# nanograv/PTMCMCSampler

Hardware: AMD Instinct MI355X
Metric: MH updates/sec (whole node) + ESS/sec, 100-d Gaussian, 64 temps x 4096 walkers per GPU (higher is better)
Workload: dtype f64

## Files before the change

### ptmcmcsampler_amd/csrc/ptmi_cov.hip

```cpp
#include <math.h>
#include <stdlib.h>

#include <type_traits>

#include "ptmi_common.h"

constexpr int WT = 7, WTILE = 16 * WT;
template <bool FUSED>
__global__ __launch_bounds__(256) void welford_kernel(const double *AM, double *mu, double *M2, double *cov, int d, int mem,
                                                     long long iter, int cov_stride_per_walker, int am_epl)
{
    constexpr int PF = 8;
    constexpr int RB = 4;
    __shared__ double sh[2][RB][2][WTILE];
    if (FUSED && blockIdx.y > blockIdx.x) return;
    const int w = (int)blockIdx.z;
    const int ti0 = (int)blockIdx.y * WTILE, tj0 = (int)blockIdx.x * WTILE;
    const int tx = (int)(threadIdx.x & 15), ty = (int)(threadIdx.x >> 4);
    const double *am = AM + (size_t)w * mem * d;
    double *muw = mu + (size_t)w * d, *M2w = M2 + (size_t)w * d * d;
    long long it = iter - mem;
    const bool reset = it == 0;

    const int role = (int)threadIdx.x / WTILE, ridx = (int)threadIdx.x % WTILE;
    const int rel = role == 0 ? ti0 + ridx : tj0 + ridx;
    const bool carrier = role < 2 && rel < d;
    double m = carrier && !reset ? muw[rel] : 0.0;

    double acc[WT][WT];
#pragma unroll
    for (int p = 0; p < WT; ++p)
#pragma unroll
        for (int r = 0; r < WT; ++r) {
            const int i = ti0 + ty + 16 * p, j = tj0 + tx + 16 * r;
            acc[p][r] = (!reset && i < d && j < d) ? M2w[(size_t)i * d + j] : 0.0;
        }
    int bsel = 0;
    for (int ii0 = 0; ii0 < mem; ii0 += PF) {
        double vpre[PF];
#pragma unroll
        for (int u = 0; u < PF; ++u) vpre[u] = (carrier && ii0 + u < mem) ? am[(size_t)(ii0 + u) * d + am_pos(rel < d ? rel : 0, am_epl)] : 0.0;
#pragma unroll
        for (int u0 = 0; u0 < PF; u0 += RB) {
            if (ii0 + u0 >= mem) break;
            if (role < 2) {
#pragma unroll
                for (int u = 0; u < RB; ++u) {
                    double df = 0.0, ev = 0.0;
                    if (carrier && ii0 + u0 + u < mem) {
                        const double v = vpre[u0 + u];
                        df = v - m;
                        if (FUSED) m = m + df * (1.0 / (double)(it + 1 + u));
                        else m += df / (double)(it + 1 + u);
                        ev = v - m;
                    }
                    if (role == 0) sh[bsel][u][0][ridx] = df;
                    else sh[bsel][u][1][ridx] = ev;
                }
            }
            __syncthreads();
#pragma unroll
            for (int u = 0; u < RB; ++u) {
                double dv[WT], evv[WT];
#pragma unroll
                for (int p = 0; p < WT; ++p) dv[p] = sh[bsel][u][0][ty + 16 * p];
#pragma unroll
                for (int r = 0; r < WT; ++r) evv[r] = sh[bsel][u][1][tx + 16 * r];
                if (ii0 + u0 + u < mem) {
#pragma unroll
                    for (int p = 0; p < WT; ++p)
#pragma unroll
                        for (int r = 0; r < WT; ++r) {
                            if (FUSED) acc[p][r] = __builtin_fma(dv[p], evv[r], acc[p][r]);
                            else acc[p][r] += dv[p] * evv[r];
                        }
                }
            }
            const int done = mem - (ii0 + u0) < RB ? mem - (ii0 + u0) : RB;
            it += done;
            bsel ^= 1;
        }
    }
    const double den = (double)(it - 1);
    double *covw = cov ? cov + (size_t)w * cov_stride_per_walker : nullptr;
#pragma unroll
    for (int p = 0; p < WT; ++p)
#pragma unroll
        for (int r = 0; r < WT; ++r) {
            const int i = ti0 + ty + 16 * p, j = tj0 + tx + 16 * r;
            if (i < d && j < d) {
                M2w[(size_t)i * d + j] = acc[p][r];
                if (covw) covw[(size_t)i * d + j] = acc[p][r] / den;
            }
        }
    if (gridDim.x == 1 && role == 0 && carrier) muw[rel] = m;
}

__device__ __forceinline__ double div_by_count(double a, double n, double r)
{
    if (__builtin_fabs(a) < 0x1p-900) return a / n;
    double q = a * r;
    double e = __builtin_fma(-n, q, a);
    q = __builtin_fma(e, r, q);
    e = __builtin_fma(-n, q, a);
    return __builtin_fma(e, r, q);
}
template <int TYN, int TXN, int PR, int PC>
__global__ __launch_bounds__(768) void welford_rows_kernel(const double *AM, double *mu, double *M2, double *cov, int d, int mem, long long iter,
                                                           int cov_stride_per_walker, int am_epl, int nwalkers)
{
#ifndef PTMI_WF_RB
#define PTMI_WF_RB 8
#endif
    constexpr int RB = PTMI_WF_RB, LW = TYN * PR > TXN * PC ? TYN * PR : TXN * PC;
    __shared__ __attribute__((aligned(16))) double sh_all[2][2][RB][2][LW];
    const int tb = (int)threadIdx.x;
    const int slot = tb < 512 ? tb >> 8 : (tb - 512) >> 7;
    const int w = 2 * (int)blockIdx.x + slot;
    const bool wact = w < nwalkers;
    double (*sh)[RB][2][LW] = sh_all[slot];
    const double *am = AM + (size_t)(wact ? w : 0) * mem * d;
    double *muw = mu + (size_t)(wact ? w : 0) * d, *M2w = M2 + (size_t)(wact ? w : 0) * d * d;
    const long long it0 = iter - mem;
    const bool reset = it0 == 0;
    const int t = tb < 512 ? (tb & 255) : 256 + ((tb - 512) & 127);
    const int nb = (mem + RB - 1) / RB;
    if (t >= 256) {
        const int rel = t - 256;
        const bool carrier = rel < d && wact;
        const int pos = am_pos(carrier ? rel : 0, am_epl);
        double m = carrier && !reset ? muw[rel] : 0.0;
        double vc[RB], vn[RB];
        auto load = [&](int b, double (&v)[RB]) {
#pragma unroll
            for (int u = 0; u < RB; ++u) {
                const int row = b * RB + u;
                v[u] = (carrier && row < mem) ? am[(size_t)row * d + pos] : 0.0;
            }
        };
        auto produce = [&](int b, const double (&v)[RB]) {
            const double nl = (double)(it0 + (long long)b * RB + 1 + (t & (RB - 1))), rl = 1.0 / nl;
#pragma unroll
            for (int u = 0; u < RB; ++u) {
                const double n = __shfl(nl, u, RB), r = __shfl(rl, u, RB);
                double df = 0.0, ev = 0.0;
#ifdef PTMI_WF_NOCARRY
                df = v[u] + n; ev = v[u] + r;
#else
                if (b * RB + u < mem) {
                    df = v[u] - m;
                    m += div_by_count(df, n, r);
                    ev = v[u] - m;
                }
#endif
                if (rel < LW) { sh[b & 1][u][0][rel] = carrier ? df : 0.0; sh[b & 1][u][1][rel] = carrier ? ev : 0.0; }
            }
        };
        load(0, vc);
        if (nb > 1) load(1, vn);
        produce(0, vc);
        __syncthreads();
        for (int b = 0; b < nb; ++b) {
            if (b + 1 < nb) {
#pragma unroll
                for (int u = 0; u < RB; ++u) vc[u] = vn[u];
                if (b + 2 < nb) load(b + 2, vn);
                produce(b + 1, vc);
            }
            __syncthreads();
        }
        if (carrier && wact) muw[rel] = m;
        return;
    }
    const int ty = t / TXN, tx = t % TXN;
    const bool live = t < TYN * TXN && wact;
    double acc[PR][PC];
#pragma unroll
    for (int p = 0; p < PR; ++p)
#pragma unroll
        for (int r = 0; r < PC; ++r) {
            const int i = ty * PR + p, j = tx * PC + r;
            acc[p][r] = (live && !reset && i < d && j < d) ? M2w[(size_t)i * d + j] : 0.0;
        }
    __syncthreads();
    for (int b = 0; b < nb; ++b) {
        if (live) {
            double dv[2][PR], ev[2][PC];
            auto rd = [&](int u, int k) {
#pragma unroll
                for (int p = 0; p < PR; ++p) dv[k][p] = sh[b & 1][u][0][ty * PR + p];
#pragma unroll
                for (int r = 0; r < PC; ++r) ev[k][r] = sh[b & 1][u][1][tx * PC + r];
            };
            auto row = [&](int k) {
#pragma unroll
                for (int p = 0; p < PR; ++p)
#pragma unroll
                    for (int r = 0; r < PC; ++r) acc[p][r] += dv[k][p] * ev[k][r];
            };
            rd(0, 0);
#pragma unroll
            for (int u = 0; u < RB; ++u) {
                if (u + 1 < RB) {
                    rd(u + 1, (u + 1) & 1);
                    __builtin_amdgcn_sched_barrier(0);
                }
                row(u & 1);
            }
        }
        __syncthreads();
    }
    if (!live) return;
    const double den = (double)(iter - 1);
    double *covw = cov ? cov + (size_t)w * cov_stride_per_walker : nullptr;
#pragma unroll
    for (int p = 0; p < PR; ++p)
#pragma unroll
        for (int r = 0; r < PC; ++r) {
            const int i = ty * PR + p, j = tx * PC + r;
            if (i < d && j < d) M2w[(size_t)i * d + j] = acc[p][r];
        }
    if (covw) {
#pragma unroll 1
        for (int e = 0; e < PR * PC; ++e) {
            const int i = ty * PR + e / PC, j = tx * PC + e % PC;
            if (i < d && j < d) covw[(size_t)i * d + j] = M2w[(size_t)i * d + j] / den;
        }
    }
}

constexpr int PS_W = 112;
constexpr int ps_rc(bool diag) { return diag ? 32 : 16; }
typedef double ps_d4 __attribute__((ext_vector_type(4)));
__host__ __device__ inline int pool_groups(int d) { return (d + 1 + PS_W - 1) / PS_W; }
static inline int pool_slab(int nwalkers, int d) { const int target = d + 1 <= PS_W ? 512 : 32; const int s = (nwalkers + target - 1) / target; return s < 1 ? 1 : s; }
struct PoolEnt { double wgt; int32_t src; int32_t pad; };
struct PoolRle { const PoolEnt *ent; const int32_t *cnt; };
typedef double ps_d2 __attribute__((ext_vector_type(2)));
constexpr int ps_nt(bool diag, int wv) { return diag ? 7 : (wv == 0 ? 13 : 12); }
__host__ __device__ constexpr int ps_t0(int wv) { return wv == 0 ? 0 : 1 + 12 * wv; }
constexpr int ps_ti(bool diag, int wv, int n) { return diag ? (n < 7 - wv ? wv : 7 - wv) : (ps_t0(wv) + n) / 7; }
constexpr int ps_tj(bool diag, int wv, int n) { return diag ? (n < 7 - wv ? wv + n : n) : (ps_t0(wv) + n) % 7; }
template <bool DIAG, int WV>
__device__ __forceinline__ void ps_mma(const double *Ab, const double *Bb, ps_d4 (&acc)[DIAG ? 7 : 13])
{
#pragma unroll
    for (int k0 = 0; k0 < ps_rc(DIAG); k0 += 4)
#pragma unroll
        for (int n = 0; n < ps_nt(DIAG, WV); ++n)
            acc[n] = __builtin_amdgcn_mfma_f64_16x16x4f64(Ab[k0 * PS_W + 16 * ps_ti(DIAG, WV, n)], Bb[k0 * PS_W + 16 * ps_tj(DIAG, WV, n)], acc[n], 0, 0, 0);
}
template <bool DIAG, int WV>
__device__ __forceinline__ void ps_store(const ps_d4 (&acc)[DIAG ? 7 : 13], double *out, int I, int J, int d, int am_epl, int g, int c)
{
#pragma unroll
    for (int n = 0; n < ps_nt(DIAG, WV); ++n) {
        const int ti = ps_ti(DIAG, WV, n), tj = ps_tj(DIAG, WV, n);
#pragma unroll
        for (int r = 0; r < 4; ++r) {
            const int pi = I * PS_W + 16 * ti + g + 4 * r, pj = J * PS_W + 16 * tj + c;
            if (pi < d && pj <= d && (!(DIAG && ti == tj) || pi <= pj)) {
                const int ci = am_inv(pi, am_epl), cj = pj < d ? am_inv(pj, am_epl) : d;
                const int lo = ci < cj ? ci : cj, hi = ci < cj ? cj : ci;
                out[(size_t)lo * (d + 1) + hi] = acc[n][r];
            }
        }
    }
}
template <bool DIAG, bool RLE, bool PAIR>
__global__ __launch_bounds__(256, 2) void pool_syrk_kernel(const double *rows, long long nrows, int d, const double *shift,
                                                                     long long rows_per_slab, double *part, int am_epl,
                                                                     int shift_epl ,
                                                                     PoolRle rl)
{
    constexpr int NTW = DIAG ? 7 : 13, NA = DIAG ? 1 : 2, PS_RC = ps_rc(DIAG), NU = PS_RC / 4;
    __shared__ double Dl[NA][2][PS_RC][PS_W];
    const int lane = (int)(threadIdx.x & 63), wave = __builtin_amdgcn_readfirstlane((int)(threadIdx.x >> 6));
    const int c = lane & 15, g = lane >> 4;
    const int ng = pool_groups(d);
    int I = (int)blockIdx.x, J = (int)blockIdx.x;
    if (!DIAG) {
        int p = (int)blockIdx.x;
        I = 0;
        while (p >= ng - 1 - I) { p -= ng - 1 - I; ++I; }
        J = I + 1 + p;
    }
    const long long beg = (long long)blockIdx.y * rows_per_slab;
    const int nlist = RLE ? rl.cnt[blockIdx.y] : (int)(beg + rows_per_slab < nrows ? rows_per_slab : nrows - beg);
    const char *slab = (const char *)(rows + beg * d);
    const PoolEnt *ent = RLE ? rl.ent + beg : nullptr;
    ps_d4 acc[NTW];
#pragma unroll
    for (int n = 0; n < NTW; ++n) acc[n] = ps_d4{0.0, 0.0, 0.0, 0.0};
    int offa[DIAG ? 1 : NTW], offb[DIAG ? 1 : NTW];
    if constexpr (!DIAG) {
#pragma unroll
        for (int n = 0; n < NTW; ++n) {
            const int t = ps_t0(wave) + n < 49 ? ps_t0(wave) + n : 48;
            offa[n] = __builtin_amdgcn_readfirstlane(16 * (t / 7));
            offb[n] = __builtin_amdgcn_readfirstlane(16 * (t % 7));
        }
    }
    const int q = 16 * wave + c, r4 = g;
    const bool stager = q < PS_W / 2;
    unsigned colb[NA][2];
    double sh[NA][2], one[NA][2];
    bool dat[NA][2];
    bool plain = true;
#pragma unroll
    for (int a2 = 0; a2 < NA; ++a2)
#pragma unroll
        for (int e = 0; e < 2; ++e) {
            const int p = (a2 == 0 ? I : J) * PS_W + 2 * q + e;
            dat[a2][e] = p < d;
            const int pc = PAIR ? (p - e < d ? p : d - 2 + e) : (p < d ? p : d - 1);
            colb[a2][e] = 8u * (unsigned)pc;
            sh[a2][e] = (stager && p < d) ? shift[am_pos(am_inv(p, am_epl), shift_epl)] : 0.0;
            one[a2][e] = p == d ? 1.0 : 0.0;
            plain = plain && (dat[a2][e] || !stager);
        }
    const bool wave_plain = __all(plain);
    const unsigned rstride = 8u * (unsigned)d;
    ps_d2 v[NA][NU];
    double wg[NU];
    int nsrc[RLE ? NU : 1];
    double nwg[RLE ? NU : 1];
    auto list = [&](int j0) {
        if constexpr (RLE) {
#pragma unroll
            for (int u = 0; u < NU; ++u) {
                const int j = j0 + 4 * u + r4, jc = j < nlist ? j : nlist - 1;
                const ps_d2 e2 = *(const ps_d2 *)(ent + jc);
                nwg[u] = e2.x;
                nsrc[u] = (int)(__double_as_longlong(e2.y) & 0xffffffffll);
            }
        }
    };
    auto fetch = [&](int j0) {
#pragma unroll
        for (int u = 0; u < NU; ++u) {
            const int j = j0 + 4 * u + r4, jc = j < nlist ? j : nlist - 1;
            const unsigned rb = (unsigned)(RLE ? nsrc[u] : jc) * rstride;
            wg[u] = j < nlist ? (RLE ? nwg[u] : 1.0) : 0.0;
#pragma unroll
            for (int a2 = 0; a2 < NA; ++a2) {
                if constexpr (PAIR) v[a2][u] = *(const ps_d2 *)(slab + (rb + colb[a2][0]));
                else {
                    v[a2][u].x = *(const double *)(slab + (rb + colb[a2][0]));
                    v[a2][u].y = *(const double *)(slab + (rb + colb[a2][1]));
                }
            }
        }
    };
    auto stage = [&](int buf) {
        if (!stager) return;
        if (wave_plain) {
#pragma unroll
            for (int a2 = 0; a2 < NA; ++a2)
#pragma unroll
                for (int u = 0; u < NU; ++u) {
                    ps_d2 x;
                    x.x = (v[a2][u].x - sh[a2][0]) * wg[u];
                    x.y = (v[a2][u].y - sh[a2][1]) * wg[u];
                    *(ps_d2 *)&Dl[a2][buf][4 * u + r4][2 * q] = x;
                }
        } else {
#pragma unroll
            for (int a2 = 0; a2 < NA; ++a2)
#pragma unroll
                for (int u = 0; u < NU; ++u) {
                    ps_d2 x;
                    x.x = (dat[a2][0] ? v[a2][u].x - sh[a2][0] : one[a2][0]) * wg[u];
                    x.y = (dat[a2][1] ? v[a2][u].y - sh[a2][1] : one[a2][1]) * wg[u];
                    *(ps_d2 *)&Dl[a2][buf][4 * u + r4][2 * q] = x;
                }
        }
    };
    if (nlist > 0) {
        list(0);
        fetch(0);
        list(PS_RC);
        stage(0);
    }
    __syncthreads();
    int buf = 0;
    for (int j0 = 0; j0 < nlist; j0 += PS_RC) {
        const bool more = j0 + PS_RC < nlist;
        if (more) {
            fetch(j0 + PS_RC);
            list(j0 + 2 * PS_RC);
        }
        const double *Ab = &Dl[0][buf][0][0] + g * PS_W + c, *Bb = &Dl[NA - 1][buf][0][0] + g * PS_W + c;
        if constexpr (DIAG) {
            switch (wave) {
            case 0: ps_mma<DIAG, 0>(Ab, Bb, acc); break;
            case 1: ps_mma<DIAG, 1>(Ab, Bb, acc); break;
            case 2: ps_mma<DIAG, 2>(Ab, Bb, acc); break;
            default: ps_mma<DIAG, 3>(Ab, Bb, acc); break;
            }
        } else {
#pragma unroll
            for (int k0 = 0; k0 < PS_RC; k0 += 4)
#pragma unroll
                for (int n = 0; n < NTW; ++n)
                    if (n < 12 || wave == 0) acc[n] = __builtin_amdgcn_mfma_f64_16x16x4f64(Ab[k0 * PS_W + offa[n]], Bb[k0 * PS_W + offb[n]], acc[n], 0, 0, 0);
        }
        if (more) stage(buf ^ 1);
        __syncthreads();
        buf ^= 1;
    }
    double *out = part + (size_t)blockIdx.y * d * (d + 1);
    if constexpr (DIAG) {
        switch (wave) {
        case 0: ps_store<DIAG, 0>(acc, out, I, J, d, am_epl, g, c); break;
        case 1: ps_store<DIAG, 1>(acc, out, I, J, d, am_epl, g, c); break;
        case 2: ps_store<DIAG, 2>(acc, out, I, J, d, am_epl, g, c); break;
        default: ps_store<DIAG, 3>(acc, out, I, J, d, am_epl, g, c); break;
        }
    } else {
#pragma unroll
        for (int n = 0; n < NTW; ++n) {
            if (!(n < 12 || wave == 0)) continue;
#pragma unroll
            for (int r = 0; r < 4; ++r) {
                const int pi = I * PS_W + offa[n] + g + 4 * r, pj = J * PS_W + offb[n] + c;
                if (pi < d && pj <= d) {
                    const int ci = am_inv(pi, am_epl), cj = pj < d ? am_inv(pj, am_epl) : d;
                    const int lo = ci < cj ? ci : cj, hi = ci < cj ? cj : ci;
                    out[(size_t)lo * (d + 1) + hi] = acc[n][r];
                }
            }
        }
    }
}

__global__ __launch_bounds__(256) void pool_rle_kernel(const AmFlag *flag, long long nrows, long long rows_per_slab, PoolEnt *ent, int32_t *cnt)
{
    constexpr int NG = 8;
    __shared__ int wsum[NG][4], base_s;
    const long long beg = (long long)blockIdx.x * rows_per_slab;
    const long long end = beg + rows_per_slab < nrows ? beg + rows_per_slab : nrows;
    const int lane = (int)(threadIdx.x & 63), wave = (int)(threadIdx.x >> 6);
    if (threadIdx.x == 0) base_s = 0;
    __syncthreads();
    for (long long r0 = beg; r0 < end; r0 += 256 * NG) {
        AmFlag f[NG];
#pragma unroll
        for (int u = 0; u < NG; ++u) { const long long r = r0 + 256 * u + threadIdx.x; f[u] = flag[r < end ? r : end - 1]; }
        unsigned long long m[NG];
#pragma unroll
        for (int u = 0; u < NG; ++u) {
            const long long r = r0 + 256 * u + threadIdx.x;
            m[u] = __ballot(r < end && (f[u] & (AMROW_NEW | AMROW_KEY)) != 0);
            if (lane == 0) wsum[u][wave] = (int)__popcll(m[u]);
        }
        __syncthreads();
        int off = base_s;
#pragma unroll
        for (int u = 0; u < NG; ++u) {
            const long long r = r0 + 256 * u + threadIdx.x;
            int mine = off + (int)__popcll(m[u] & ((1ull << lane) - 1ull));
            for (int k = 0; k < wave; ++k) mine += wsum[u][k];
            if ((m[u] >> lane) & 1ull) ent[beg + mine].src = (int32_t)(r - beg);
            off += wsum[u][0] + wsum[u][1] + wsum[u][2] + wsum[u][3];
        }
        __syncthreads();
        if (threadIdx.x == 0) base_s = off;
        __syncthreads();
    }
    const int n = base_s;
    if (threadIdx.x == 0) cnt[blockIdx.x] = n;
    for (int j0 = 0; j0 < n; j0 += 256 * NG) {
        int here[NG], next[NG];
#pragma unroll
        for (int u = 0; u < NG; ++u) {
            const int j = j0 + 256 * u + (int)threadIdx.x, jc = j < n ? j : n - 1;
            here[u] = ent[beg + jc].src;
            next[u] = jc + 1 < n ? ent[beg + jc + 1].src : (int)(end - beg);
        }
#pragma unroll
        for (int u = 0; u < NG; ++u) {
            const int j = j0 + 256 * u + (int)threadIdx.x;
            if (j < n) ent[beg + j].wgt = det_sqrt((double)((long long)next[u] - (long long)here[u]));
        }
    }
}

__global__ __launch_bounds__(128) void am_expand_kernel(double *AM, const AmFlag *flag, int d, int cu, int w0, long long it_lo, long long it_hi,
                                                        long long base)
{
    const int w = w0 + (int)blockIdx.x;
    const AmFlag *fw = flag + (size_t)w * cu;
    double *aw = AM + (size_t)w * cu * d;
    long long it0 = it_lo;
    while (it0 > base && !(fw[it0 % cu] & (AMROW_NEW | AMROW_KEY))) --it0;
    for (int i = (int)threadIdx.x; i < d; i += (int)blockDim.x) {
        double x = aw[(size_t)(it0 % cu) * d + i];
        for (long long it = it0 + 1; it <= it_hi; ++it) {
            const int ring = (int)(it % cu);
            if (fw[ring] & (AMROW_NEW | AMROW_KEY)) x = aw[(size_t)ring * d + i];
            else if (it >= it_lo) aw[(size_t)ring * d + i] = x;
        }
    }
}
__global__ void pool_reduce_kernel(const double *part, int nslab, int d, double *Tsum)
{
    const long long idx = (long long)blockIdx.x * blockDim.x + threadIdx.x;
    const int ld = d + 1;
    if (idx >= (long long)d * ld) return;
    const int i = (int)(idx / ld), j = (int)(idx % ld);
    if (j < i) return;
    const size_t st = (size_t)d * ld;
    double sum = 0.0;
    int s = 0;
    for (; s + 32 <= nslab; s += 32) {
        double v[32];
#pragma unroll
        for (int u = 0; u < 32; ++u) v[u] = part[(size_t)(s + u) * st + idx];
#pragma unroll
        for (int u = 0; u < 32; ++u) sum += v[u];
    }
    for (; s + 8 <= nslab; s += 8) {
        double v[8];
#pragma unroll
        for (int u = 0; u < 8; ++u) v[u] = part[(size_t)(s + u) * st + idx];
#pragma unroll
        for (int u = 0; u < 8; ++u) sum += v[u];
    }
    for (; s < nslab; ++s) sum += part[(size_t)s * st + idx];
    Tsum[idx] = sum;
}
__global__ void pool_finish_kernel(const double *Tsum, const double *shift, int shift_epl, double *mu, double *M2, double *cov, int d, int first,
                                   double nb, double f , double gw , double den)
{
    const long long idx = (long long)blockIdx.x * blockDim.x + threadIdx.x;
    if (idx >= (long long)d * d) return;
    const int i = (int)(idx / d), j = (int)(idx % d), ld = d + 1;
    if (j < i) return;
    const double ti = Tsum[(size_t)i * ld + d], tj = Tsum[(size_t)j * ld + d];
    const double M2b = Tsum[(size_t)i * ld + j] - (ti * tj) / nb;
    double m;
    if (first) m = M2b;
    else m = (M2[idx] + M2b) + ((ti / nb) * (tj / nb)) * f;
    M2[idx] = m;
    M2[(size_t)j * d + i] = m;
    const double cv = m / den;
    cov[idx] = cv;
    cov[(size_t)j * d + i] = cv;
    if (i == j) mu[i] = first ? shift[am_pos(i, shift_epl)] + ti / nb : mu[i] + (ti / nb) * gw;
}

__global__ void welford_mean_kernel(const double *AM, double *mu, int d, int mem, long long iter, int fused, int am_epl)
{
    const int w = (int)blockIdx.y;
    const int j = (int)(blockIdx.x * blockDim.x + threadIdx.x);
    if (j >= d) return;
    const double *am = AM + (size_t)w * mem * d;
    long long it = iter - mem;
    double m = it == 0 ? 0.0 : mu[(size_t)w * d + j];
    for (int ii = 0; ii < mem; ++ii) {
        it += 1;
        const double df = am[(size_t)ii * d + am_pos(j, am_epl)] - m;
        if (fused) m = m + df * (1.0 / (double)it);
        else m += df / (double)it;
    }
    mu[(size_t)w * d + j] = m;
}

__global__ void de_update_kernel(double *DE, const double *AM, int d, int de_size, int mem, int head, int W, int pooled, int ld, int epl, int am_epl)
{
    const int r = (int)blockIdx.x;
    const int wc = (int)blockIdx.y;
    const int skip = mem > de_size ? mem - de_size : 0;
    if (r < skip) return;
    const int phys = (head + (r - skip)) % de_size;
    const int src_w = pooled ? r % W : wc;
    const double *src = AM + ((size_t)src_w * mem + r) * d;
    double *dst = DE + ((size_t)wc * de_size + phys) * ld;
    for (int j = (int)threadIdx.x; j < ld; j += (int)blockDim.x) {
        int i = j;
        if (epl) {
            const int e = 2 * (j / 8) + (j & 1);
            i = e < epl ? ((j & 7) >> 1) + 4 * e : d;
        }
        dst[j] = i < d ? src[am_pos(i, am_epl)] : 0.0;
    }
}

hipError_t ptmi_pool_scratch_alloc(ptmi_engine *h)
{
    const ptmi_config &c = h->cfg;
    const int SL = pool_slab(c.nwalkers, c.ndim), nslab = (c.nwalkers + SL - 1) / SL;
    hipError_t e = hipMalloc((void **)&h->d_pool_part, sizeof(double) * (size_t)nslab * c.ndim * (c.ndim + 1));
    if (e == hipSuccess) e = hipMalloc((void **)&h->d_pool_T, sizeof(double) * (size_t)c.ndim * (c.ndim + 1));
    if (h->buf.AMflag) {
        const size_t nrows = (size_t)c.nwalkers * c.cov_update;
        if (e == hipSuccess) e = hipMalloc((void **)&h->d_rle_ent, sizeof(PoolEnt) * nrows);
        if (e == hipSuccess) e = hipMalloc((void **)&h->d_rle_cnt, sizeof(int32_t) * (size_t)nslab);
    }
    return e;
}

extern "C" {

int ptmi_update_cov(ptmi_handle h, int64_t iter) { return ptmi_update_cov_on(h, iter, nullptr, nullptr, nullptr); }

int ptmi_set_am_buffers(ptmi_handle h, double *AM, double *AMaux, uint64_t *AMflag)
{
    if (!h) return fail(PTMI_EINVAL, "NULL handle");
    if (!AM || !h->buf.AM) return fail(PTMI_EINVAL, "the handle was created without an AM buffer, or AM is NULL");
    if ((AMaux != nullptr) != (h->buf.AMaux != nullptr) || (AMflag != nullptr) != (h->buf.AMflag != nullptr))
        return fail(PTMI_EINVAL, "AMaux / AMflag must be given exactly when the handle was created with them");
    h->buf.AM = AM; h->buf.AMaux = AMaux; h->buf.AMflag = AMflag;
    return PTMI_OK;
}

int ptmi_update_cov_on(ptmi_handle hh, int64_t iter, void *stream, const double *AM_in, const uint64_t *AMflag_in)
{
    if (!hh) return fail(PTMI_EINVAL, "NULL handle");
    ptmi_engine view = *hh;
    if (stream) view.stream = (hipStream_t)stream;
    if (AM_in) { view.buf.AM = const_cast<double *>(AM_in); view.buf.AMflag = const_cast<uint64_t *>(AMflag_in); }
    ptmi_engine *h = &view;
    struct Back { ptmi_engine *to, *from; ~Back() { to->side = from->side; to->side_go = from->side_go; to->side_done = from->side_done; } } back{hh, h};
    const ptmi_config &c = h->cfg;
    if (c.temp0 != 0) return PTMI_OK;
    if (!h->buf.AM || !h->buf.mu || !h->buf.M2 || !h->buf.cov) return fail(PTMI_EINVAL, "AM/mu/M2/cov buffers missing");
    if (iter < c.cov_update || iter % c.cov_update) return fail(PTMI_EINVAL, "iter must be a positive multiple of cov_update");
    const int d = c.ndim, nt = (d + WTILE - 1) / WTILE;
    if (c.cov_per_walker) {
        if (d <= 100)
            hipLaunchKernelGGL((welford_rows_kernel<25, 10, 4, 10>), dim3((c.nwalkers + 1) / 2), dim3(768), 0, h->stream, (const double *)h->buf.AM,
                               h->buf.mu, h->buf.M2, h->buf.cov, d, c.cov_update, (long long)iter, d * d, am_row_epl(h->G, h->EPL), c.nwalkers);
        else
        hipLaunchKernelGGL(welford_kernel<false>, dim3(nt, nt, c.nwalkers), dim3(256), 0, h->stream, (const double *)h->buf.AM,
                           h->buf.mu, h->buf.M2, h->buf.cov, d, c.cov_update, (long long)iter, d * d, am_row_epl(h->G, h->EPL));
        if (nt > 1)
            hipLaunchKernelGGL(welford_mean_kernel, dim3((d + 63) / 64, c.nwalkers), dim3(64), 0, h->stream, (const double *)h->buf.AM,
                               h->buf.mu, d, c.cov_update, (long long)iter, 0, am_row_epl(h->G, h->EPL));
    } else {
        const int W = c.nwalkers, SL = pool_slab(W, d), nslab = (W + SL - 1) / SL, ng = pool_groups(d);
        const long long nrows = (long long)W * c.cov_update;
        const bool first = iter == c.cov_update;
        const double *shift = first ? (const double *)h->buf.AM : (const double *)h->buf.mu;
        hipStream_t diag_stream = h->stream;
        const bool rle = h->buf.AMflag != nullptr, pair = d % 2 == 0;
        const PoolRle pr = {(const PoolEnt *)h->d_rle_ent, h->d_rle_cnt};
        const long long rps = (long long)SL * c.cov_update;
        if (rps * d * 8 >= (1ll << 32)) return fail(PTMI_EUNSUPPORTED, "pooled statistics: a slab of %d walkers x %d rows x %d parameters exceeds 4 GB", SL, c.cov_update, d);
        const int aepl = am_row_epl(h->G, h->EPL), sepl = first ? am_row_epl(h->G, h->EPL) : 0;
        if (rle) hipLaunchKernelGGL(pool_rle_kernel, dim3(nslab), dim3(256), 0, h->stream, (const AmFlag *)h->buf.AMflag, nrows, rps, (PoolEnt *)h->d_rle_ent,
                                    h->d_rle_cnt);
        auto syrk = [&](auto diag, dim3 grid, hipStream_t st) {
            constexpr bool DG = decltype(diag)::value;
            const void *fn = rle ? (pair ? (const void *)pool_syrk_kernel<DG, true, true> : (const void *)pool_syrk_kernel<DG, true, false>)
                                 : (pair ? (const void *)pool_syrk_kernel<DG, false, true> : (const void *)pool_syrk_kernel<DG, false, false>);
            const double *rows = (const double *)h->buf.AM;
            long long nr = nrows, rp = rps;
            int dd = d, ae = aepl, se = sepl;
            double *part = h->d_pool_part;
            PoolRle prl = pr;
            void *args[] = {&rows, &nr, &dd, (void *)&shift, &rp, &part, &ae, &se, &prl};
            return hipLaunchKernel(fn, grid, dim3(256), args, 0, st);
        };
        if (ng > 1) {
            if (!h->side) {
                HIPCHK(hipStreamCreateWithFlags(&h->side, hipStreamNonBlocking));
                HIPCHK(hipEventCreateWithFlags(&h->side_go, hipEventDisableTiming));
                HIPCHK(hipEventCreateWithFlags(&h->side_done, hipEventDisableTiming));
            }
            HIPCHK(hipEventRecord(h->side_go, h->stream));
            HIPCHK(hipStreamWaitEvent(h->side, h->side_go, 0));
            HIPCHK(syrk(std::false_type{}, dim3(ng * (ng - 1) / 2, nslab), h->stream));
            diag_stream = h->side;
        }
        HIPCHK(syrk(std::true_type{}, dim3(ng, nslab), diag_stream));
        if (ng > 1) {
            HIPCHK(hipEventRecord(h->side_done, h->side));
            HIPCHK(hipStreamWaitEvent(h->stream, h->side_done, 0));
        }
        const long long nel = (long long)d * (d + 1);
        hipLaunchKernelGGL(pool_reduce_kernel, dim3((unsigned)((nel + 63) / 64)), dim3(64), 0, h->stream, (const double *)h->d_pool_part, nslab, d,
                           h->d_pool_T);
        const double nb = (double)W * (double)c.cov_update, nprev = (double)W * (double)(iter - c.cov_update);
        hipLaunchKernelGGL(pool_finish_kernel, dim3((unsigned)(((long long)d * d + 255) / 256)), dim3(256), 0, h->stream, (const double *)h->d_pool_T,
                           shift, first ? am_row_epl(h->G, h->EPL) : 0, h->buf.mu, h->buf.M2, h->buf.cov, d, first ? 1 : 0, nb, nprev * nb / (nprev + nb), nb / (nprev + nb),
                           nprev + nb - 1.0);
    }
    HIPCHK(hipGetLastError());
    return PTMI_OK;
}

int ptmi_am_expand(ptmi_handle h, int32_t w0, int32_t nw, int64_t iter_lo, int64_t iter_hi)
{
    if (!h) return fail(PTMI_EINVAL, "NULL handle");
    const ptmi_config &c = h->cfg;
    if (!h->buf.AMflag || !h->buf.AM) return PTMI_OK;
    if (w0 < 0 || nw < 0 || w0 + nw > c.nwalkers) return fail(PTMI_EINVAL, "walkers [%d, %d) of %d", w0, w0 + nw, c.nwalkers);
    const long long base = iter_hi > 0 ? ((long long)(iter_hi - 1) / c.cov_update) * c.cov_update : 0;
    if (iter_lo < base || iter_hi < iter_lo || iter_hi - iter_lo >= c.cov_update)
        return fail(PTMI_EINVAL, "iterations %lld..%lld are not inside the covariance period that starts at %lld (with AM row flags the ring keeps "
                                 "the rows of the current period only)", (long long)iter_lo, (long long)iter_hi, base);
    if (nw == 0) return PTMI_OK;
    hipLaunchKernelGGL(am_expand_kernel, dim3((unsigned)nw), dim3(128), 0, h->stream, h->buf.AM, (const AmFlag *)h->buf.AMflag, c.ndim, c.cov_update,
                       (int)w0, (long long)iter_lo, (long long)iter_hi, base);
    HIPCHK(hipGetLastError());
    return PTMI_OK;
}

int ptmi_update_de(ptmi_handle h)
{
    if (!h) return fail(PTMI_EINVAL, "NULL handle");
    const ptmi_config &c = h->cfg;
    if (!h->buf.DE) return PTMI_OK;
    if (!h->buf.AM) return fail(PTMI_EINVAL, "DE update needs the AM buffer on this GPU");
    const int wc = c.cov_per_walker ? c.nwalkers : 1;
    hipLaunchKernelGGL(de_update_kernel, dim3(c.cov_update, wc), dim3(64), 0, h->stream, h->buf.DE, (const double *)h->buf.AM,
                       c.ndim, c.de_size, c.cov_update, h->de_head, c.nwalkers, c.cov_per_walker ? 0 : 1,
                       de_row_ld(h->G, h->EPL, c.ndim), h->G == 4 ? h->EPL : 0, am_row_epl(h->G, h->EPL));
    HIPCHK(hipGetLastError());
    const int adv = c.cov_update < c.de_size ? c.cov_update : c.de_size;
    h->de_head = (h->de_head + adv) % c.de_size;
    return PTMI_OK;
}

int ptmi_set_de_head(ptmi_handle h, int32_t head)
{
    if (!h) return fail(PTMI_EINVAL, "NULL handle");
    if (head < 0 || head >= h->cfg.de_size) return fail(PTMI_EINVAL, "head %d outside the ring of %d rows", head, h->cfg.de_size);
    h->de_head = head;
    return PTMI_OK;
}

}
```

Baseline: 37.78 billion.

## Use per-dimension precomputed 8-wide tile plans for single-group pooled SYRK diagonal

Adds compile-time tile plans, one per dimension bucket of 8. Each plan assigns the MFMA tiles of the triangular covariance block to the four waves using 8x8 half-tiles and per-tile ownership masks. This replaces the fixed 16-wide 7x7 diagonal tiling when the whole dimension fits in one group. The aim is to cut wasted MFMA work on padded and duplicated triangular tiles and to balance work across waves. Costs are many extra kernel instantiations, precomputed LDS fragment offsets held in registers, and a target attribute that disables LDS load/store merging, which may hurt LDS throughput.

```diff
diff --git a/ptmcmcsampler_amd/csrc/ptmi_cov.hip b/ptmcmcsampler_amd/csrc/ptmi_cov.hip
--- a/ptmcmcsampler_amd/csrc/ptmi_cov.hip
+++ b/ptmcmcsampler_amd/csrc/ptmi_cov.hip
@@ -2,8 +2,10 @@
 #include <stdlib.h>
 
 #include <type_traits>
+#include <utility>
 
 #include "ptmi_common.h"
+#include "ptmi_pool_plan.h"
 
 constexpr int WT = 7, WTILE = 16 * WT;
 template <bool FUSED>
@@ -267,13 +269,103 @@
         }
     }
 }
-template <bool DIAG, bool RLE, bool PAIR>
-__global__ __launch_bounds__(256, 2) void pool_syrk_kernel(const double *rows, long long nrows, int d, const double *shift,
+constexpr PcTile pc_tile(int m, int wv, int n) { return pc_plan[m].t[pc_plan[m].w0[wv] + n]; }
+constexpr int pc_nt(int m, int wv) { return pc_plan[m].w0[wv + 1] - pc_plan[m].w0[wv]; }
+constexpr int pc_set(int m, int wv, int s) { const PcTile t = pc_tile(m, wv, s / 2); return s % 2 ? 16 * t.b0 + t.b1 : 16 * t.a0 + t.a1; }
+constexpr bool pc_first(int m, int wv, int s)
+{
+    for (int j = 0; j < s; ++j)
+        if (pc_set(m, wv, j) == pc_set(m, wv, s)) return false;
+    return true;
+}
+constexpr int pc_rank(int m, int wv, int s)
+{
+    const int ns = 2 * pc_nt(m, wv);
+    int rank = 0;
+    for (int i = 0; i < ns; ++i) {
+        if (s < ns && pc_set(m, wv, i) == pc_set(m, wv, s)) return rank;
+        rank += pc_first(m, wv, i) ? 1 : 0;
+    }
+    return rank;
+}
+template <int M, int WV, int S>
+__device__ __forceinline__ void pc_frag1(int (&fo)[PC_FRAG_BUDGET], int g, int c)
+{
+    constexpr int set = pc_set(M, WV, S), r = pc_rank(M, WV, S);
+    static_assert(r < PC_FRAG_BUDGET, "a wave reads more distinct fragments than the budget");
+    if constexpr (pc_first(M, WV, S)) {
+        fo[r] = g * PS_W + (c & 7) + 8 * ((c & 8) ? set % 16 : set / 16);
+        asm volatile("" : "+v"(fo[r]));
+    }
+}
+template <int M, int WV, int... S>
+__device__ __forceinline__ void pc_frags(int (&fo)[PC_FRAG_BUDGET], int g, int c, std::integer_sequence<int, S...>)
+{
+    (pc_frag1<M, WV, S>(fo, g, c), ...);
+}
+template <int M, int WV>
+__device__ __forceinline__ void pc_frags(int (&fo)[PC_FRAG_BUDGET], int g, int c)
+{
+    pc_frags<M, WV>(fo, g, c, std::make_integer_sequence<int, 2 * pc_nt(M, WV)>{});
+}
+template <int M, int WV, int N>
+__device__ __forceinline__ void pc_mma1(const double *D, const int (&fo)[PC_FRAG_BUDGET], ps_d4 &acc)
+{
+    constexpr int ra = pc_rank(M, WV, 2 * N), rb = pc_rank(M, WV, 2 * N + 1);
+    acc = __builtin_amdgcn_mfma_f64_16x16x4f64(D[fo[ra]], D[fo[rb]], acc, 0, 0, 0);
+}
+template <int M, int WV, int... N>
+__device__ __forceinline__ void pc_mma(const double *D, const int (&fo)[PC_FRAG_BUDGET], ps_d4 (&acc)[PC_NTW], std::integer_sequence<int, N...>)
+{
+#pragma unroll
+    for (int k0 = 0; k0 < ps_rc(true); k0 += 4)
+        (pc_mma1<M, WV, N>(D + k0 * PS_W, fo, acc[N]), ...);
+}
+template <int M, int WV>
+__device__ __forceinline__ void pc_mma(const double *D, const int (&fo)[PC_FRAG_BUDGET], ps_d4 (&acc)[PC_NTW])
+{
+    pc_mma<M, WV>(D, fo, acc, std::make_integer_sequence<int, pc_nt(M, WV)>{});
+}
+template <int M, int WV, int N>
+__device__ __forceinline__ void pc_store1(const ps_d4 &acc, double *out, int d, int am_epl, int g, int c)
+{
+    constexpr PcTile t = pc_tile(M, WV, N);
+    const bool hi = (c & 8) != 0;
+#pragma unroll
+    for (int r = 0; r < 4; ++r) {
+        const int ax = r < 2 ? t.a0 : t.a1, by = hi ? t.b1 : t.b0;
+        const bool own = ((hi ? t.own >> 1 : t.own) >> (2 * (r >> 1)) & 1) != 0;
+        const int pi = 8 * ax + g + 4 * (r & 1), pj = 8 * by + (c & 7);
+        if (own && pi <= d && pj <= d && (ax != by || pi <= pj)) {
+            const int ci = pi < d ? am_inv(pi, am_epl) : d, cj = pj < d ? am_inv(pj, am_epl) : d;
+            const int lo = ci < cj ? ci : cj, up = ci < cj ? cj : ci;
+            if (lo < d) out[(size_t)lo * (d + 1) + up] = acc[r];
+        }
+    }
+}
+template <int M, int WV, int... N>
+__device__ __forceinline__ void pc_store(const ps_d4 (&acc)[PC_NTW], double *out, int d, int am_epl, int g, int c, std::integer_sequence<int, N...>)
+{
+    (pc_store1<M, WV, N>(acc[N], out, d, am_epl, g, c), ...);
+}
+template <int M, int WV>
+__device__ __forceinline__ void pc_store(const ps_d4 (&acc)[PC_NTW], double *out, int d, int am_epl, int g, int c)
+{
+    pc_store<M, WV>(acc, out, d, am_epl, g, c, std::make_integer_sequence<int, pc_nt(M, WV)>{});
+}
+#if defined(__HIP_DEVICE_COMPILE__)
+#define PS_PLAIN_LDS_READS __attribute__((target("no-load-store-opt")))
+#else
+#define PS_PLAIN_LDS_READS
+#endif
+template <bool DIAG, bool RLE, bool PAIR, int M = 0>
+PS_PLAIN_LDS_READS __global__ __launch_bounds__(256, 2) void pool_syrk_kernel(const double *rows, long long nrows, int d, const double *shift,
                                                                      long long rows_per_slab, double *part, int am_epl,
                                                                      int shift_epl ,
                                                                      PoolRle rl)
 {
-    constexpr int NTW = DIAG ? 7 : 13, NA = DIAG ? 1 : 2, PS_RC = ps_rc(DIAG), NU = PS_RC / 4;
+    static_assert(M == 0 || DIAG, "a plan is for the only macro tile");
+    constexpr int NTW = M ? PC_NTW : DIAG ? 7 : 13, NA = DIAG ? 1 : 2, PS_RC = ps_rc(DIAG), NU = PS_RC / 4;
     __shared__ double Dl[NA][2][PS_RC][PS_W];
     const int lane = (int)(threadIdx.x & 63), wave = __builtin_amdgcn_readfirstlane((int)(threadIdx.x >> 6));
     const int c = lane & 15, g = lane >> 4;
@@ -301,6 +393,15 @@
             offb[n] = __builtin_amdgcn_readfirstlane(16 * (t % 7));
         }
     }
+    int fo[PC_FRAG_BUDGET] = {};
+    if constexpr (M != 0) {
+        switch (wave) {
+        case 0: pc_frags<M, 0>(fo, g, c); break;
+        case 1: pc_frags<M, 1>(fo, g, c); break;
+        case 2: pc_frags<M, 2>(fo, g, c); break;
+        default: pc_frags<M, 3>(fo, g, c); break;
+        }
+    }
     const int q = 16 * wave + c, r4 = g;
     const bool stager = q < PS_W / 2;
     unsigned colb[NA][2];
@@ -391,7 +492,15 @@
             list(j0 + 2 * PS_RC);
         }
         const double *Ab = &Dl[0][buf][0][0] + g * PS_W + c, *Bb = &Dl[NA - 1][buf][0][0] + g * PS_W + c;
-        if constexpr (DIAG) {
+        if constexpr (M != 0) {
+            const double *Db = &Dl[0][buf][0][0];
+            switch (wave) {
+            case 0: pc_mma<M, 0>(Db, fo, acc); break;
+            case 1: pc_mma<M, 1>(Db, fo, acc); break;
+            case 2: pc_mma<M, 2>(Db, fo, acc); break;
+            default: pc_mma<M, 3>(Db, fo, acc); break;
+            }
+        } else if constexpr (DIAG) {
             switch (wave) {
             case 0: ps_mma<DIAG, 0>(Ab, Bb, acc); break;
             case 1: ps_mma<DIAG, 1>(Ab, Bb, acc); break;
@@ -410,7 +519,14 @@
         buf ^= 1;
     }
     double *out = part + (size_t)blockIdx.y * d * (d + 1);
-    if constexpr (DIAG) {
+    if constexpr (M != 0) {
+        switch (wave) {
+        case 0: pc_store<M, 0>(acc, out, d, am_epl, g, c); break;
+        case 1: pc_store<M, 1>(acc, out, d, am_epl, g, c); break;
+        case 2: pc_store<M, 2>(acc, out, d, am_epl, g, c); break;
+        default: pc_store<M, 3>(acc, out, d, am_epl, g, c); break;
+        }
+    } else if constexpr (DIAG) {
         switch (wave) {
         case 0: ps_store<DIAG, 0>(acc, out, I, J, d, am_epl, g, c); break;
         case 1: ps_store<DIAG, 1>(acc, out, I, J, d, am_epl, g, c); break;
@@ -433,6 +549,14 @@
         }
     }
 }
+template <int... MM>
+static const void *pool_plan_kernel(int m, bool rle, bool pair, std::integer_sequence<int, MM...>)
+{
+    static const void *const fn[PC_MMAX][4] = {{(const void *)pool_syrk_kernel<true, false, false, MM + 1>, (const void *)pool_syrk_kernel<true, false, true, MM + 1>,
+                                                (const void *)pool_syrk_kernel<true, true, false, MM + 1>, (const void *)pool_syrk_kernel<true, true, true, MM + 1>}...};
+    return fn[m - 1][2 * (rle ? 1 : 0) + (pair ? 1 : 0)];
+}
+static const void *pool_plan_kernel(int m, bool rle, bool pair) { return pool_plan_kernel(m, rle, pair, std::make_integer_sequence<int, PC_MMAX>{}); }
 
 __global__ __launch_bounds__(256) void pool_rle_kernel(const AmFlag *flag, long long nrows, long long rows_per_slab, PoolEnt *ent, int32_t *cnt)
 {
@@ -655,6 +779,7 @@
             constexpr bool DG = decltype(diag)::value;
             const void *fn = rle ? (pair ? (const void *)pool_syrk_kernel<DG, true, true> : (const void *)pool_syrk_kernel<DG, true, false>)
                                  : (pair ? (const void *)pool_syrk_kernel<DG, false, true> : (const void *)pool_syrk_kernel<DG, false, false>);
+            if (DG && ng == 1) fn = pool_plan_kernel((d + 8) / 8, rle, pair);
             const double *rows = (const double *)h->buf.AM;
             long long nr = nrows, rp = rps;
             int dd = d, ae = aepl, se = sepl;
diff --git a/ptmcmcsampler_amd/csrc/ptmi_pool_plan.h b/ptmcmcsampler_amd/csrc/ptmi_pool_plan.h
--- /dev/null
+++ b/ptmcmcsampler_amd/csrc/ptmi_pool_plan.h
@@ -0,0 +1,82 @@
+#pragma once
+struct PcTile { signed char a0, a1, b0, b1, own; };
+struct PcPlan { int nt; int w0[5]; PcTile t[28]; };
+constexpr int PC_MMAX = 14, PC_NTW = 7, PC_FRAG_BUDGET = 9;
+constexpr PcPlan pc_plan[PC_MMAX + 1] = {
+    {0, {0, 0, 0, 0, 0}, {}},
+    {1, {0, 1, 1, 1, 1}, {
+        {0, 1, 0, 1, 1},
+    }},
+    {1, {0, 1, 1, 1, 1}, {
+        {0, 1, 0, 1, 11},
+    }},
+    {2, {0, 1, 2, 2, 2}, {
+        {0, 1, 0, 1, 11},
+        {0, 2, 1, 2, 14},
+    }},
+    {3, {0, 1, 2, 3, 3}, {
+        {0, 1, 0, 1, 11},
+        {0, 1, 2, 3, 15},
+        {2, 3, 2, 3, 11},
+    }},
+    {5, {0, 2, 3, 4, 5}, {
+        {1, 3, 0, 2, 15}, {1, 3, 1, 3, 11},
+        {0, 2, 0, 2, 11},
+        {0, 4, 1, 3, 12},
+        {0, 4, 2, 4, 14},
+    }},
+    {6, {0, 2, 4, 5, 6}, {
+        {4, 5, 0, 1, 15}, {4, 5, 4, 5, 11},
+        {0, 1, 0, 1, 11}, {0, 1, 2, 3, 15},
+        {2, 3, 4, 5, 15},
+        {2, 3, 2, 3, 11},
+    }},
+    {7, {0, 2, 4, 6, 7}, {
+        {0, 3, 3, 4, 15}, {1, 6, 3, 6, 15},
+        {0, 5, 1, 5, 15}, {2, 3, 2, 5, 15},
+        {1, 2, 1, 4, 15}, {4, 5, 4, 6, 15},
+        {0, 2, 0, 6, 15},
+    }},
+    {10, {0, 3, 6, 8, 10}, {
+        {2, 3, 4, 5, 15}, {2, 3, 6, 7, 15}, {4, 5, 6, 7, 15},
+        {0, 1, 0, 1, 11}, {0, 1, 2, 3, 15}, {2, 3, 2, 3, 11},
+        {6, 7, 0, 1, 15}, {6, 7, 6, 7, 11},
+        {4, 5, 0, 1, 15}, {4, 5, 4, 5, 11},
+    }},
+    {12, {0, 3, 6, 9, 12}, {
+        {2, 7, 2, 8, 15}, {2, 7, 5, 6, 15}, {5, 6, 0, 6, 15},
+        {0, 2, 0, 1, 15}, {0, 2, 3, 4, 15}, {3, 4, 4, 6, 15},
+        {1, 5, 4, 5, 15}, {1, 7, 1, 7, 11}, {1, 8, 6, 8, 15},
+        {3, 5, 1, 3, 11}, {3, 5, 7, 8, 11}, {7, 8, 0, 4, 15},
+    }},
+    {15, {0, 4, 8, 12, 15}, {
+        {0, 1, 0, 1, 11}, {0, 1, 2, 3, 15}, {0, 1, 8, 9, 15}, {8, 9, 8, 9, 11},
+        {2, 3, 2, 3, 11}, {4, 5, 2, 3, 15}, {4, 5, 4, 5, 11}, {4, 5, 8, 9, 15},
+        {0, 1, 4, 5, 15}, {6, 7, 0, 1, 15}, {6, 7, 4, 5, 15}, {6, 7, 6, 7, 11},
+        {2, 3, 6, 7, 15}, {2, 3, 8, 9, 15}, {6, 7, 8, 9, 15},
+    }},
+    {17, {0, 5, 9, 13, 17}, {
+        {3, 10, 1, 3, 15}, {3, 10, 2, 8, 15}, {3, 10, 4, 9, 15}, {4, 9, 2, 7, 15}, {4, 9, 6, 9, 15},
+        {0, 4, 0, 5, 15}, {0, 8, 2, 9, 15}, {0, 8, 8, 10, 7}, {2, 3, 5, 7, 15},
+        {0, 1, 1, 7, 15}, {0, 6, 3, 6, 15}, {1, 2, 2, 6, 15}, {6, 7, 7, 8, 15},
+        {1, 4, 4, 8, 15}, {1, 5, 5, 9, 15}, {5, 10, 6, 8, 7}, {5, 10, 7, 10, 15},
+    }},
+    {21, {0, 6, 11, 16, 21}, {
+        {4, 5, 0, 1, 15}, {4, 5, 4, 5, 11}, {4, 5, 6, 7, 15}, {4, 5, 8, 9, 15}, {8, 9, 6, 7, 15}, {8, 9, 8, 9, 11},
+        {2, 3, 2, 3, 11}, {2, 3, 4, 5, 15}, {2, 3, 10, 11, 15}, {10, 11, 4, 5, 15}, {10, 11, 10, 11, 11},
+        {0, 1, 6, 7, 15}, {0, 1, 8, 9, 15}, {0, 1, 10, 11, 15}, {10, 11, 6, 7, 15}, {10, 11, 8, 9, 15},
+        {0, 1, 0, 1, 11}, {2, 3, 0, 1, 15}, {2, 3, 6, 7, 15}, {2, 3, 8, 9, 15}, {6, 7, 6, 7, 11},
+    }},
+    {23, {0, 6, 12, 18, 23}, {
+        {0, 4, 2, 7, 15}, {0, 4, 4, 6, 15}, {2, 5, 5, 7, 15}, {2, 5, 8, 9, 15}, {3, 11, 7, 11, 15}, {8, 9, 4, 11, 15},
+        {1, 6, 1, 11, 15}, {1, 6, 3, 5, 15}, {1, 11, 2, 4, 15}, {2, 3, 2, 12, 15}, {3, 5, 4, 10, 15}, {3, 8, 3, 9, 15},
+        {0, 5, 0, 11, 15}, {0, 5, 3, 12, 15}, {1, 7, 7, 12, 15}, {1, 7, 9, 10, 15}, {2, 10, 6, 10, 15}, {9, 10, 0, 9, 15},
+        {0, 8, 1, 8, 15}, {6, 7, 6, 8, 15}, {6, 12, 9, 12, 15}, {10, 12, 4, 8, 15}, {10, 12, 11, 12, 7},
+    }},
+    {28, {0, 7, 14, 21, 28}, {
+        {2, 3, 0, 1, 15}, {2, 3, 2, 3, 11}, {2, 3, 4, 5, 15}, {2, 3, 10, 11, 15}, {4, 5, 4, 5, 11}, {10, 11, 0, 1, 15}, {10, 11, 10, 11, 11},
+        {2, 3, 6, 7, 15}, {2, 3, 8, 9, 15}, {2, 3, 12, 13, 15}, {6, 7, 8, 9, 15}, {6, 7, 12, 13, 15}, {8, 9, 0, 1, 15}, {12, 13, 0, 1, 15},
+        {0, 1, 0, 1, 11}, {0, 1, 4, 5, 15}, {4, 5, 10, 11, 15}, {6, 7, 0, 1, 15}, {6, 7, 4, 5, 15}, {6, 7, 6, 7, 11}, {6, 7, 10, 11, 15},
+        {8, 9, 4, 5, 15}, {8, 9, 8, 9, 11}, {8, 9, 10, 11, 15}, {8, 9, 12, 13, 15}, {12, 13, 4, 5, 15}, {12, 13, 10, 11, 15}, {12, 13, 12, 13, 11},
+    }},
+};
```

After: 37.29 billion. 0.987x the previous value.
